# UoL-SignalProcessingGroup/SMC-NUTS

Measured on AMD Instinct MI355X. Metric: leapfrog-steps/sec, higher is better.
Workload: dtype f64

## Files before the change

### include/smcnuts_hip.h

```cpp
#ifndef SMCNUTS_HIP_H
#define SMCNUTS_HIP_H

#include <stddef.h>
#include <stdint.h>

#ifdef __cplusplus
extern "C" {
#endif

typedef struct smcn_ctx smcn_ctx;

#define SMCN_MODEL_GAUSS 0
#define SMCN_MODEL_ARMA 1
#define SMCN_MODEL_PRMWCD 2
#define SMCN_MODEL_HOST 3
#define SMCN_MODEL_GLM 4
#define SMCN_MODEL_HGLM 5
#define SMCN_MODEL_CATEGORICAL 6
#define SMCN_MODEL_ORDINAL 7
#define SMCN_MODEL_MLGLM 8
#define SMCN_MODEL_WGLM 9
#define SMCN_MODEL_OGLM 10

#define SMCN_LKERNEL_FORWARD 0
#define SMCN_LKERNEL_GAUSSIAN 1

#define SMCN_FLAG_TAPE_OVERFLOW 1

int smcn_version(void);
const char* smcn_last_error(const smcn_ctx* ctx);

int smcn_ctx_create(smcn_ctx** out, int device_id, int64_t n_particles, int64_t particle_base,
                    int model_id, const double* model_data, int64_t model_data_len);
void smcn_ctx_destroy(smcn_ctx* ctx);
int smcn_dim(const smcn_ctx* ctx);
int smcn_constrained_dim(const smcn_ctx* ctx);
int smcn_fused_transitions(const smcn_ctx* ctx);
int smcn_set_stream(smcn_ctx* ctx, void* hip_stream);
int smcn_synchronize(smcn_ctx* ctx);

int smcn_set_seed(smcn_ctx* ctx, uint64_t seed);

int smcn_set_state(smcn_ctx* ctx, const double* x, const double* logw);
int smcn_get_state(smcn_ctx* ctx, double* x, double* logw, double* wn);
int smcn_get_proposal(smcn_ctx* ctx, double* r, double* x_new, double* r_new, double* logw_new);
int smcn_set_momentum(smcn_ctx* ctx, const double* r);
int smcn_set_proposal(smcn_ctx* ctx, const double* r, const double* x_new, const double* r_new);

int smcn_target_eval(smcn_ctx* ctx, const double* x, int64_t M, double phi, double* logp,
                     double* grad, double* lpri, double* llik);
int smcn_target_constrain(smcn_ctx* ctx, const double* x, int64_t M, double* out);

int smcn_init_particles_std_normal(smcn_ctx* ctx, double phi);
int smcn_init_weights(smcn_ctx* ctx, double phi, const double* logq0);

int smcn_normalise_partials(smcn_ctx* ctx, double out[4]);
int smcn_normalise_apply(smcn_ctx* ctx, double loglik);
int smcn_normalise(smcn_ctx* ctx, double* loglik, double* ess);

int smcn_moment_sums(smcn_ctx* ctx, const double* mean_or_null, double* sums);

int smcn_resample_multinomial(smcn_ctx* ctx, const double* u, double loglik, double log_n_total,
                              int64_t iteration, int64_t* idx_out);
#define SMCN_RESAMPLE_MULTINOMIAL 0
#define SMCN_RESAMPLE_SYSTEMATIC 1
int smcn_set_resample_scheme(smcn_ctx* ctx, int scheme);
int smcn_set_wide_eval(smcn_ctx* ctx, int on);
int smcn_set_phase_paths(smcn_ctx* ctx, int on);
int smcn_set_tree_align(smcn_ctx* ctx, int n);
int smcn_get_wave_iterations(smcn_ctx* ctx, uint32_t* out, int64_t n);
int smcn_set_lane_grid(smcn_ctx* ctx, int64_t waves);
int smcn_set_lane_segments(smcn_ctx* ctx, int segments);

int smcn_set_nuts_cap(smcn_ctx* ctx, int doublings, int widen);
int smcn_nuts_parked(smcn_ctx* ctx, int64_t* parked);
int smcn_set_nuts_requeue(smcn_ctx* ctx, int doublings);

int smcn_propose_nuts(smcn_ctx* ctx, double step_size, double phi, int max_depth, double delta_max,
                      int64_t iteration, const double* tape, const int64_t* tape_off);
int smcn_get_tree_stats(smcn_ctx* ctx, int32_t* nleap, int32_t* depth, int32_t* ndraws, int32_t* flags);
int smcn_last_leapfrogs(smcn_ctx* ctx, int64_t* total);
int smcn_get_density_parts(smcn_ctx* ctx, double* lpri0, double* llik0, double* lpri1, double* llik1);

int smcn_reweight(smcn_ctx* ctx, int lkernel);
int smcn_accept_reject(smcn_ctx* ctx, double phi, const double* u, int64_t iteration);
int smcn_reweight_asymptotic(smcn_ctx* ctx, double phi_old, double phi_new);
int smcn_set_logw_density_ratio(smcn_ctx* ctx, double phi_num, double phi_den);

int smcn_set_lkernel_values(smcn_ctx* ctx, const double* L, const double* q);

int smcn_gauss_lkernel_sums(smcn_ctx* ctx, const double* shift, double* sums);
int smcn_gauss_lkernel_logpdf(smcn_ctx* ctx, const double* mu_x, const double* m0, const double* B,
                              const double* U, double c0);
int smcn_gauss_lkernel_device(smcn_ctx* ctx, double info[4]);
int smcn_gauss_lkernel_buffers(smcn_ctx* ctx, int world, void** local_dev, void** gathered_dev);
int smcn_gauss_lkernel_stage(smcn_ctx* ctx, int stage, int world, double n_total, double info[4] );

int smcn_temper_partials(smcn_ctx* ctx, double phi_old, double phi_new, double out[4]);
int smcn_temper_bisect(smcn_ctx* ctx, double phi_old, double target, double* phi, int* status);
int smcn_temper_bisect_pass(smcn_ctx* ctx, int pass, double phi_old);
int smcn_temper_bisect_buffers(smcn_ctx* ctx, int world, void** local, void** gathered);
int smcn_temper_bisect_decide(smcn_ctx* ctx, int pass, int world, double target, double phi_old);
int smcn_temper_bisect_result(smcn_ctx* ctx, double* phi, int* status);

int smcn_eval_proposed_parts(smcn_ctx* ctx, int which);

int smcn_commit(smcn_ctx* ctx, int64_t* n_moved);

int smcn_fast_begin(smcn_ctx* ctx, int64_t K, int save_history, int world);
int smcn_fast_buffers(smcn_ctx* ctx, void** local_partials, void** gathered, int* nq);
int smcn_set_resample_uniforms(smcn_ctx* ctx, const double* u);
int smcn_step_begin(smcn_ctx* ctx, int64_t k);
int smcn_step_finish(smcn_ctx* ctx, int64_t k, int world, int rank, double n_total, double step_size,
                     double phi, int max_depth, double delta_max, int lkernel, int last,
                     const double* tape, const int64_t* tape_off);
int smcn_fast_read(smcn_ctx* ctx, double* hist, double* x_saved, double* logw_saved);
int smcn_fast_read_from(smcn_ctx* ctx, double* hist, double* x_saved, double* logw_saved, int64_t k_from);
int smcn_history_download(smcn_ctx* ctx, int64_t k_from, int64_t k_to, double* x_saved, double* logw_saved);
int smcn_fuse_begin(smcn_ctx* ctx, int Bmax, int world);
int smcn_fuse_buffers(smcn_ctx* ctx, void** local_partials, void** gathered, int* nq);
int smcn_fuse_run(smcn_ctx* ctx, int64_t k0, int B, int world, int rank, double n_total, double step_size,
                  double phi, int max_depth, double delta_max, int decided);
// ... 133 lines not shown
```

### smcnuts_amd/_capi.py

```python
import ctypes as C
import os

import numpy as np

from . import build as _build

MODEL_GAUSS, MODEL_ARMA, MODEL_PRMWCD, MODEL_HOST = 0, 1, 2, 3
MODEL_GLM = 4
MODEL_HGLM = 5
MODEL_CATEGORICAL = 6
MODEL_ORDINAL = 7
MODEL_MLGLM = 8
MODEL_WGLM = 9
MODEL_OGLM = 10
HOST_TARGET_FN = C.CFUNCTYPE(C.c_int, C.c_void_p, C.c_int64, C.c_int, C.POINTER(C.c_double), C.c_int,
                             C.POINTER(C.c_double), C.POINTER(C.c_double), C.POINTER(C.c_double),
                             C.POINTER(C.c_double))
LKERNEL_FORWARD, LKERNEL_GAUSSIAN = 0, 1

_dp = C.POINTER(C.c_double)
_ip = C.POINTER(C.c_int32)
_lp = C.POINTER(C.c_int64)
_ctx = C.c_void_p

# ... 14 lines not shown
    "smcn_set_momentum": ([_ctx, _dp], C.c_int),
    "smcn_set_proposal": ([_ctx, _dp, _dp, _dp], C.c_int),
    "smcn_target_eval": ([_ctx, _dp, C.c_int64, C.c_double, _dp, _dp, _dp, _dp], C.c_int),
    "smcn_target_constrain": ([_ctx, _dp, C.c_int64, _dp], C.c_int),
    "smcn_init_particles_std_normal": ([_ctx, C.c_double], C.c_int),
    "smcn_init_weights": ([_ctx, C.c_double, _dp], C.c_int),
    "smcn_normalise_partials": ([_ctx, _dp], C.c_int),
    "smcn_normalise_apply": ([_ctx, C.c_double], C.c_int),
    "smcn_normalise": ([_ctx, _dp, _dp], C.c_int),
    "smcn_moment_sums": ([_ctx, _dp, _dp], C.c_int),
    "smcn_resample_multinomial": ([_ctx, _dp, C.c_double, C.c_double, C.c_int64, _lp], C.c_int),
    "smcn_propose_nuts": ([_ctx, C.c_double, C.c_double, C.c_int, C.c_double, C.c_int64, _dp, _lp], C.c_int),
    "smcn_get_tree_stats": ([_ctx, _ip, _ip, _ip, _ip], C.c_int),
    "smcn_last_leapfrogs": ([_ctx, _lp], C.c_int),
    "smcn_get_density_parts": ([_ctx, _dp, _dp, _dp, _dp], C.c_int),
    "smcn_set_lkernel_values": ([_ctx, _dp, _dp], C.c_int),
    "smcn_reweight": ([_ctx, C.c_int], C.c_int),
    "smcn_accept_reject": ([_ctx, C.c_double, _dp, C.c_int64], C.c_int),
    "smcn_reweight_asymptotic": ([_ctx, C.c_double, C.c_double], C.c_int),
    "smcn_set_logw_density_ratio": ([_ctx, C.c_double, C.c_double], C.c_int),
    "smcn_gauss_lkernel_sums": ([_ctx, _dp, _dp], C.c_int),
    "smcn_gauss_lkernel_logpdf": ([_ctx, _dp, _dp, _dp, _dp, C.c_double], C.c_int),
    "smcn_gauss_lkernel_device": ([_ctx, _dp], C.c_int),
    "smcn_gauss_lkernel_buffers": ([_ctx, C.c_int, C.POINTER(C.c_void_p), C.POINTER(C.c_void_p)], C.c_int),
    "smcn_gauss_lkernel_stage": ([_ctx, C.c_int, C.c_int, C.c_double, _dp], C.c_int),
    "smcn_set_nuts_cap": ([_ctx, C.c_int, C.c_int], C.c_int),
    "smcn_set_nuts_requeue": ([_ctx, C.c_int], C.c_int),
    "smcn_nuts_parked": ([_ctx, C.POINTER(C.c_int64)], C.c_int),
    "smcn_temper_partials": ([_ctx, C.c_double, C.c_double, _dp], C.c_int),
    "smcn_temper_bisect": ([_ctx, C.c_double, C.c_double, C.POINTER(C.c_double), C.POINTER(C.c_int)], C.c_int),
    "smcn_temper_bisect_pass": ([_ctx, C.c_int, C.c_double], C.c_int),
    "smcn_temper_bisect_buffers": ([_ctx, C.c_int, C.POINTER(C.c_void_p), C.POINTER(C.c_void_p)], C.c_int),
    "smcn_temper_bisect_decide": ([_ctx, C.c_int, C.c_int, C.c_double, C.c_double], C.c_int),
    "smcn_temper_bisect_result": ([_ctx, C.POINTER(C.c_double), C.POINTER(C.c_int)], C.c_int),
    "smcn_eval_proposed_parts": ([_ctx, C.c_int], C.c_int),
    "smcn_commit": ([_ctx, _lp], C.c_int),
    "smcn_fast_begin": ([_ctx, C.c_int64, C.c_int, C.c_int], C.c_int),
    "smcn_fast_buffers": ([_ctx, C.POINTER(C.c_void_p), C.POINTER(C.c_void_p), C.POINTER(C.c_int)], C.c_int),
    "smcn_set_resample_uniforms": ([_ctx, _dp], C.c_int),
    "smcn_step_begin": ([_ctx, C.c_int64], C.c_int),
    "smcn_step_finish": ([_ctx, C.c_int64, C.c_int, C.c_int, C.c_double, C.c_double, C.c_double, C.c_int,
                          C.c_double, C.c_int, C.c_int, _dp, _lp], C.c_int),
    "smcn_fast_read": ([_ctx, _dp, _dp, _dp], C.c_int),
    "smcn_fast_read_from": ([_ctx, _dp, _dp, _dp, C.c_int64], C.c_int),
    "smcn_history_download": ([_ctx, C.c_int64, C.c_int64, _dp, _dp], C.c_int),
    "smcn_fuse_begin": ([_ctx, C.c_int, C.c_int], C.c_int),
    "smcn_fuse_buffers": ([_ctx, C.POINTER(C.c_void_p), C.POINTER(C.c_void_p), C.POINTER(C.c_int)], C.c_int),
    "smcn_fuse_run": ([_ctx, C.c_int64, C.c_int, C.c_int, C.c_int, C.c_double, C.c_double, C.c_double, C.c_int,
                       C.c_double, C.c_int], C.c_int),
    "smcn_set_resample_scheme": ([_ctx, C.c_int], C.c_int),
    "smcn_set_wide_eval": ([_ctx, C.c_int], C.c_int),
    "smcn_set_phase_paths": ([_ctx, C.c_int], C.c_int),
    "smcn_set_tree_align": ([_ctx, C.c_int], C.c_int),
    "smcn_get_wave_iterations": ([_ctx, C.POINTER(C.c_uint32), C.c_int64], C.c_int),
    "smcn_set_lane_grid": ([_ctx, C.c_int64], C.c_int),
    "smcn_set_lane_segments": ([_ctx, C.c_int], C.c_int),
    "smcn_set_host_target": ([_ctx, HOST_TARGET_FN, C.c_void_p], C.c_int),
    "smcn_moment_sums_of": ([_ctx, _dp, C.c_int, _dp, _dp], C.c_int),
    "smcn_block_resample_local": ([_ctx, C.c_int64], C.c_int),
    "smcn_block_launch": ([_ctx, C.c_int64, C.c_int, C.c_double, C.c_double, C.c_int, C.c_double], C.c_int),
    "smcn_block_post": ([_ctx, C.c_int64, C.c_int, C.c_int], C.c_int),
    "smcn_block_partials_get": ([_ctx, C.c_int, _dp], C.c_int),
    "smcn_block_partials_set": ([_ctx, C.c_int, C.c_int, _dp], C.c_int),
    "smcn_block_stats": ([_ctx, C.c_int64, C.c_int, C.c_int, C.c_int, C.c_double, C.c_double, C.c_int], C.c_int),
    "smcn_block_wait": ([_ctx, C.c_int, C.POINTER(C.c_int), C.POINTER(C.c_int)], C.c_int),
    "smcn_block_commit": ([_ctx, C.c_int64, C.c_int], C.c_int),
    "smcn_set_block_post": ([_ctx, C.c_int], C.c_int),
    "smcn_block_ess": ([_ctx, C.c_int, _dp], C.c_int),
    "smcn_fuse_decide": ([_ctx, C.c_int64, C.c_int, C.c_int, C.c_double, C.c_double, C.POINTER(C.c_int)], C.c_int),
    "smcn_fuse_finish": ([_ctx, C.c_int64, C.c_int, C.c_int, C.c_int, C.c_double, C.c_double,
                          C.POINTER(C.c_int)], C.c_int),
    "smcn_partials_get": ([_ctx, _dp], C.c_int),
    "smcn_partials_set_gathered": ([_ctx, _dp, C.c_int], C.c_int),
    "smcn_timers": ([_ctx, _dp, C.c_int], C.c_int),
    "smcn_selftest_math": ([_ctx, _dp, C.c_int64, _dp], C.c_int),
    "smcn_measure_peaks": ([_ctx, _dp], C.c_int),
    "smcn_selftest_wide": ([_ctx, C.c_int, _dp, C.c_int64, _dp], C.c_int),
    "smcn_selftest_recur": ([_ctx, _dp, C.c_int64, _dp], C.c_int),
    "smcn_device_cache_trim": ([C.c_int, C.POINTER(C.c_int64), C.POINTER(C.c_int64)], C.c_int),
    "smcn_debug_profile": ([_ctx, C.POINTER(C.c_uint64), C.c_int], C.c_int),
    "smcn_bench_resample": ([_ctx, C.c_int, C.c_int64, _dp], C.c_int),
    "smcn_comm_unique_id": ([C.c_char_p], C.c_int),
    "smcn_comm_init": ([_ctx, C.c_int, C.c_int, C.c_char_p], C.c_int),
    "smcn_comm_destroy": ([_ctx], C.c_int),
    "smcn_comm_info": ([_ctx, C.POINTER(C.c_int)], C.c_int),
    "smcn_comm_allgather": ([_ctx, C.c_void_p, C.c_void_p, C.c_int64], C.c_int),
    "smcn_comm_allgather_host": ([_ctx, _dp, C.c_int64, _dp], C.c_int),
    "smcn_comm_alltoallv": ([_ctx, C.c_void_p, _lp, C.c_void_p, _lp, C.c_int], C.c_int),
    "smcn_buf_get": ([_ctx, C.c_void_p, C.c_int64, _dp], C.c_int),
    "smcn_buf_set": ([_ctx, C.c_void_p, C.c_int64, _dp], C.c_int),
    "smcn_buf_copy": ([_ctx, C.c_void_p, C.c_void_p, C.c_int64], C.c_int),
    "smcn_gres_begin": ([_ctx, C.c_int, _dp], C.c_int),
    "smcn_gres_buffers": ([_ctx] + [C.POINTER(C.c_void_p)] * 6, C.c_int),
    "smcn_gres_plan": ([_ctx, C.c_int, C.c_int, _dp, C.c_int64, _ip], C.c_int),
    "smcn_gres_set_order": ([_ctx, _ip], C.c_int),
    "smcn_gres_reserve": ([_ctx, C.c_int64], C.c_int),
    "smcn_gres_serve": ([_ctx, C.c_int, C.c_int, C.c_int64], C.c_int),
    "smcn_gres_finish": ([_ctx, C.c_int, _dp], C.c_int),
    "smcn_pointwise_dims": ([_ctx, _lp, C.POINTER(C.c_int)], C.c_int),
    "smcn_pointwise_loglik": ([_ctx, _dp, C.c_int64, _dp], C.c_int),
    "smcn_pointwise_partials": ([_ctx, _dp, _dp, C.c_int64, _dp], C.c_int),
    "smcn_pointwise_last_ms": ([_ctx, _dp], C.c_int),
    "smcn_psis_candidates": ([_ctx, _dp, _dp, C.c_int64, C.c_double, C.c_int64, _dp], C.c_int),
    "smcn_psis_body": ([_ctx, _dp, _dp, C.c_int64, C.c_double, C.c_int64, _dp, _dp], C.c_int),
    "smcn_psis_fit": ([_ctx, _dp, _dp, C.c_int64, C.c_double, C.c_int64, _dp], C.c_int),
    "smcn_psis_loo": ([_ctx, _dp, _dp, C.c_int64, _dp, _dp], C.c_int),
# ... 504 lines not shown
```

### smcnuts_amd/csrc/smcn_api.hip

```cpp
#include <hip/hip_runtime.h>

#include <dlfcn.h>

#include <cmath>
#include <cstdio>
#include <cstring>
#include <chrono>
#include <cstdlib>
#include <map>
#include <mutex>
#include <string>
#include <thread>
#include <unordered_map>
#include <vector>

#include "smcn_ctx.hpp"
#include "smcn_nuts.hpp"
#include "smcn_nuts_wave.hpp"
#include "smcn_nuts_fin.hpp"
#include "smcn_nuts2.hpp"
#include "smcn_nuts3.hpp"
#include "smcn_temper.hpp"
#include "smcn_nuts_host.hpp"
#include "smcn_weights.hpp"
// ... 441 lines not shown
    *out = c;
    return 0;
}

void smcn_ctx_destroy(smcn_ctx* c) {
    if (!c) return;
    (void)hipSetDevice(c->device);
    (void)stream_wait(c->stream);
    free_all(c);
    delete c;
}

int smcn_dim(const smcn_ctx* c) { return c ? c->D : -1; }
int smcn_constrained_dim(const smcn_ctx* c) { return c ? c->Dc : -1; }
int smcn_fused_transitions(const smcn_ctx* c) { return c ? (c->fused_ok ? 1 : 0) : -1; }

int smcn_set_stream(smcn_ctx* c, void* s) {
    CHECK_CTX(c);
    HIPC(c, stream_wait(c->stream));
    if (c->own_stream && c->stream) pool_give(c->device, c->stream);
    c->stream = (hipStream_t)s;
    c->own_stream = false;
    return 0;
}

int smcn_synchronize(smcn_ctx* c) {
    CHECK_CTX(c);
    HIPC(c, stream_wait(c->stream));
    return 0;
}

int smcn_set_resample_scheme(smcn_ctx* c, int scheme) {
    CHECK_CTX(c);
    if (scheme != 0 && scheme != 1) FAIL(c, "smcn_set_resample_scheme: 0 (multinomial) or 1 (systematic)");
    c->resample_scheme = scheme;
    return 0;
}
int smcn_set_wide_eval(smcn_ctx* c, int on) {
    CHECK_CTX(c);
    if (on != 0 && on != 1) FAIL(c, "smcn_set_wide_eval: 0 or 1");
    c->wide_eval = on;
    return 0;
}
int smcn_set_phase_paths(smcn_ctx* c, int on) {
    CHECK_CTX(c);
    if (on != 0 && on != 1) FAIL(c, "smcn_set_phase_paths: 0 or 1");
    c->phase_paths = on;
    return 0;
}
int smcn_set_tree_align(smcn_ctx* c, int n) {
    CHECK_CTX(c);
    if (n != 1 && n != 2 && n != 4 && n != 8) FAIL(c, "smcn_set_tree_align: 1, 2, 4 or 8");
    c->tree_align = n;
    return 0;
}
int smcn_get_wave_iterations(smcn_ctx* c, uint32_t* out, int64_t n) {
    CHECK_CTX(c);
    if (!out || n < 0) FAIL(c, "smcn_get_wave_iterations: bad arguments");
    if (n > c->wave_iters_n) FAIL(c, "smcn_get_wave_iterations: the last lane-kernel launch had fewer wavefronts (or there was none)");
    HIPC(c, stream_wait(c->stream));
    if (n > 0) HIPC(c, hipMemcpy(out, c->wave_iters, sizeof(uint32_t) * n, hipMemcpyDeviceToHost));
    return 0;
}
int smcn_set_block_post(smcn_ctx* c, int mode) {
    CHECK_CTX(c);
    if (mode != 0 && mode != 1) FAIL(c, "smcn_set_block_post: 0 (separate launches) or 1 (fused)");
    c->block_post_mode = mode;
    return 0;
}

int smcn_set_lane_grid(smcn_ctx* c, int64_t waves) {
    CHECK_CTX(c);
    c->lane_grid_cap = waves;
    return 0;
}

int smcn_set_lane_segments(smcn_ctx* c, int segments) {
    CHECK_CTX(c);
    if (segments < 0 || segments > 64) FAIL(c, "smcn_set_lane_segments: 0 (auto) .. 64");
    c->lane_segments = segments;
    return 0;
}

int smcn_set_host_target(smcn_ctx* c, smcn_host_target_fn fn, void* user) {
    CHECK_CTX(c);
    if (c->model != SMCN_MODEL_HOST) FAIL(c, "smcn_set_host_target: the context was not created with SMCN_MODEL_HOST");
    c->host_fn = fn;
    c->host_user = user;
    return 0;
}

int smcn_set_seed(smcn_ctx* c, uint64_t seed) {
    CHECK_CTX(c);
    c->seed = seed;
    return 0;
}

}

bool smcn_host::has_constrain_pass(const smcn_ctx* c) {
    return c->model == SMCN_MODEL_HGLM || c->model == SMCN_MODEL_ORDINAL || c->model == SMCN_MODEL_MLGLM;
}
void smcn_host::launch_constrain_pass(smcn_ctx* c, const double* x, double* out, int64_t M, int64_t Np, int64_t si,
                                      int64_t sc) {
    if (c->model == SMCN_MODEL_ORDINAL)
        ord_constrain_kernel<<<grid_for(M, 256), 256, 0, c->stream>>>(x, out, M, Np, c->D, (int)c->reg.p, si, sc);
// ... 815 lines not shown
    c->kin_valid = false;
    if (a.resume_in) {
        a.kin0 = nullptr; a.kin1 = nullptr; a.moved = nullptr;
    }
    HIPC(c, hipMemsetAsync(c->queue, 0, sizeof(unsigned int) * 16, c->stream));
    return timed_launch(c, [&] { nuts_kernel<Model, HBM, TP><<<(int)blocks, kNutsBlock, lds, c->stream>>>(a); });
}

static int reset_records(smcn_ctx* c, int64_t cap, int D) {
    c->rec_cap = 0;
    HIPC(c, stream_wait(c->stream));
    c->in_rec.release();
    c->out_rec.release();
    HIPC(c, c->in_rec.reset(c->N * cap * n2_in_doubles(D)));
    HIPC(c, c->out_rec.reset(c->N * cap * n2_out_doubles(D)));
    c->rec_cap = cap;
    return 0;
}
template <class Model, bool TAPE, int LC, int LF>
static int launch_nuts3(smcn_ctx* c, Nuts2Args a, const double* tape_d, const int64_t* tape_off_d, bool fuse_reweight,
                        int B, double* gen_x, double* gen_logw, double* cnt, int phase) {
    constexpr int D = Model::D, VP = n2_vp(D);
    const int64_t N = c->N;
    if (TAPE && B != 1) FAIL(c, "nuts3: recorded tapes replay one transition at a time");
    if (phase == 2 && B > c->rec_cap) FAIL(c, "nuts3: post without a launch");
    if (B > c->rec_cap) {
        const int cap = c->fuse_max > B ? c->fuse_max : B;
        if (int rc = reset_records(c, cap, D)) return rc;
    }
    const size_t lds = (size_t)n3_lds_bytes<Model>(LC, LF);
    int64_t blocks = (N + kN3Block - 1) / kN3Block;
    const int64_t resident = (int64_t)c->num_cu * 4;
    if (c->lane_grid_cap > 0 && blocks > c->lane_grid_cap) blocks = c->lane_grid_cap;
    else if (c->lane_grid_cap == 0 && blocks > resident) blocks = resident;
    if (((N + blocks - 1) / blocks + 63) / 64 > kN3ReadyWords) blocks = (N + kN3Block - 1) / kN3Block;
    if (int rc = grow(c, c->n2_ovf, blocks * kN3Block * 2 * (int64_t)n3_ovf_pairs(D, LC, LF))) return rc;
    a.ovf = c->n2_ovf;
    if (phase != 2) {
        if (int rc = grow(c, c->wave_iters, blocks)) return rc;
        a.wave_iters = c->wave_iters;
        a.tree_align = c->tree_align;
        c->wave_iters_n = blocks;
        if (c->momentum_set && B != 1) FAIL(c, "nuts3: caller-supplied momenta go with single transitions");
        nuts3_prep_kernel<D><<<grid_for(N * B, 256), 256, 0, c->stream>>>(c->x, c->momentum_set ? c->r : nullptr, c->r,
                                                                         c->in_rec, N, c->base, c->seed, a.iter, B, tape_d,
                                                                         tape_off_d);
        c->momentum_set = false;
        a.in = c->in_rec;
        a.out = c->out_rec;
        a.B = B;
        a.logw0 = (fuse_reweight && B > 1) ? c->logw : nullptr;
        a.wide = (c->wide_eval ? 1 : 0) | 2;
        a.phase_paths = c->phase_paths;
        const bool queued = blocks * kN3Block < N;
        a.seg_len = 0;
        a.seg_tail = 0;
        a.seg_align = 4;
        if (queued) {
            const int64_t per_wave = (N + blocks - 1) / blocks, words = (per_wave + 63) / 64;
            int nseg = c->lane_segments > 0 ? c->lane_segments : 4;
            if (nseg > B) nseg = (int)B;
            while (nseg > 1 && nseg * words > kN3ReadyWords) --nseg;
            a.seg_tail = 0;
            if (nseg > 1) a.seg_len = (int)((B + nseg - 1) / nseg);
            int64_t segs = a.seg_len > 0 ? (B + a.seg_len - 1) / a.seg_len : 1;
            const int64_t last_len = B - (segs - 1) * a.seg_len;
            if (segs > 1 && last_len >= 2 && (segs + 1) * words <= kN3ReadyWords) {
                a.seg_tail = (int)((2 * last_len + 2) / 5 > 0 ? (2 * last_len + 2) / 5 : 1);
                ++segs;
            }
            const int64_t hw = N * (segs - 1) * 2 * (n2_vp(D) / 2 + 1);
            if (int rc = grow(c, c->handover, hw)) return rc;
            a.handover = c->handover;
        }
        const void* const kfn = queued ? (const void*)nuts3_kernel<Model, TAPE, LC, LF, true, 1>
                                       : (const void*)nuts3_kernel<Model, TAPE, LC, LF, false, 1>;
        HIPC(c, hipFuncSetAttribute(kfn, hipFuncAttributeMaxDynamicSharedMemorySize, (int)lds));
        const int rc = timed_launch(c, [&] {
            if (queued) nuts3_kernel<Model, TAPE, LC, LF, true, 1><<<(int)blocks, kN3Block, lds, c->stream>>>(a);
            else nuts3_kernel<Model, TAPE, LC, LF, false, 1><<<(int)blocks, kN3Block, lds, c->stream>>>(a);
        });
        if (rc) return rc;
    }
    if (phase == 1) return 0;
    c->streamed_g = 0;
    if (const int slots = (phase == 2 && fuse_reweight && gen_x && gen_logw && cnt) ? block_stream_slots(c, B) : 0) {
        const int g = partials_grid(c, B);
        if ((int64_t)g * B * (gen_block_nq(D) + 2) > part_doubles(c->D)) FAIL(c, "nuts3: block partials do not fit");
        double* const cntpart = c->part + (int64_t)g * B * gen_block_nq(D);
        auto stream = [&](auto kr) {
            block_stream_kernel<D, decltype(kr)::value><<<dim3(g, B), kRedBlock, 0, c->stream>>>(
                c->out_rec, c->in_rec, c->x, c->logw, c->x_new, c->r_new, c->lpri0, c->llik0, c->lpri1, c->llik1,
                c->nleap, c->depth, c->ndraws, c->flags, c->logw_new, c->x_next, c->logw_next, gen_x, gen_logw, N, B,
                c->cmodel, c->part, cntpart);
        };
        if (slots == 4) stream(std::integral_constant<int, 4>{});
        else stream(std::integral_constant<int, 8>{});
        HIPC(c, hipGetLastError());
        c->streamed_g = g;
        return 0;
    }
    nuts2_post_kernel<D><<<grid_for(N, 256), 256, 0, c->stream>>>(
        c->out_rec, c->in_rec, c->x, fuse_reweight ? c->logw : nullptr, c->x_new, c->r_new, c->lpri0, c->llik0,
        c->lpri1, c->llik1, c->nleap, c->depth, c->ndraws, c->flags, fuse_reweight ? c->logw_new : nullptr, gen_x,
        gen_logw, cnt, N, c->D, VP, B, (fuse_reweight && B > 1) ? 1 : 0, 1);
    HIPC(c, hipGetLastError());
// ... 1413 lines not shown
```

### smcnuts_amd/csrc/smcn_ctx.hpp

```cpp
#pragma once
#include <hip/hip_runtime.h>

#include <chrono>
#include <cstdint>
#include <cstdlib>
#include <string>
#include <vector>

#include "../../include/smcnuts_hip.h"
#include "smcn_comm.hpp"
#include "smcn_devbuf.hpp"
#include "smcn_draw_plan.hpp"
#include "smcn_regdata.hpp"

namespace smcn { struct PwArgs; }

namespace smcn_host __attribute__((visibility("hidden"))) {
using namespace smcn;
constexpr int kTimerRing = 512;

struct CacheMem { static int alloc(void** p, size_t bytes); static void free(void* p, bool synced); };
struct PinnedMem {
    static int alloc(void** p, size_t bytes) { return (int)hipHostMalloc(p, bytes); }
    static void free(void* p, bool) { (void)hipHostFree(p); }
// ... 71 lines not shown
    bool own_stream = false;
    uint64_t seed = 0;
    std::string err;
    std::vector<double> mdata_h;
    RegLayout reg;

    Buf<double> mdata, x, x_new, x_tmp, r, r_new;
    Buf<double> logw, logw_new, wn, work;
    Buf<double> lpri0, llik0, lpri1, llik1, Lg, qv;
    Buf<double> scan_local, ttot, toff, part, scal;
    Buf<double> glk_buf;
    Buf<double> glk_xchg;
    int glk_world = 0;
    int nuts_jcap = 0, nuts_wide2 = 1;
    Buf<double> nuts_resume;
    Buf<unsigned int> nuts_pend;
    Buf<unsigned int> nuts_mq;
    Buf<double> nuts_mq_rec;
    int nuts_mq_b = 0;
    bool nuts_mq_used = false;
    bool nuts_mq_ok = false;
    int64_t nuts_parked = 0;
    Buf<double> stage;
    Buf<double> stage2;
    Buf<double> cstage;
    Buf<int32_t> nleap, depth, ndraws, flags;
    Buf<int64_t> idx;
    Buf<unsigned int> queue;
    Buf<double> kin0;
    Buf<double> kin1;
    Buf<int32_t> moved_i;
    bool kin_valid = false;
    bool r_pm = false, r_new_pm = false;
    Buf<unsigned long long> prof;
    Buf<double> tape_d;
    Buf<int64_t> tape_off_d;
    bool momentum_set = false, lg_set = false, q_set = false, u_set = false;
    Buf<double> hist, ss, lp, gath, hist_x, hist_logw;
    Buf<double> u_res;
    Buf<double> in_rec, out_rec;
    Buf<double> nuts_scratch;
    int64_t fast_K = -1;
    bool fast_hist = false;
    int fuse_max = 0;
    int64_t rec_cap = 0;
    int resample_scheme = 0;
    bool fused_ok = false;
    bool lane_kernel = false;
    int64_t arma_T = 0;
    Buf<double> tb_state, tb_part, tb_local, tb_gath;
    int tb_world = 0, tb_blocks = 0;
    int wide_eval = 1;
    int phase_paths = 1;
    int tree_align = 4;
    Buf<unsigned int> wave_iters;
    int64_t wave_iters_n = 0;
    int64_t lane_grid_cap = 0;
    int lane_segments = 0;
    Buf<unsigned long long> handover;
    bool plain_block = false;
    int block_post_mode = 1;
    bool cnt_zeroed = false;
    int streamed_g = 0;
    double block_phi = 1.0;
    struct { int64_t k0 = -1; int B = 0; double n_total = 0.0, phi = 0.0; } tail_combined;
    Buf<double> x_next, logw_next;
    uint64_t api_seq = 0;
    struct { uint64_t seq = 0; int64_t k0 = -1; int B = 0; } next;
    ncclComm_t comm = nullptr;
    int comm_rank = 0, comm_world = 1;
    Buf<double> g_ttot_all, g_toff_all, g_keys, g_keys_send, g_keys_recv, g_rows_send, g_rows_recv;
    Buf<int32_t> g_dest, g_order;
    int64_t g_serve_cap = 0;
    int g_world = 0;
    smcn_host_target_fn host_fn = nullptr;
    void* host_user = nullptr;
    Buf<double> hc_vec, hc_sc, hc_gp, hc_gl;
    Buf<int32_t> hc_st;
    std::vector<double> hx, hlp, hll, hgp, hgl;
    Buf<double> n2_ovf;
    Buf<double> ss_scratch;
    DevBuf<double, PinnedMem> rows_h;
    DevBuf<double, PinnedMem> hist_h;
    bool hist_h_valid = false;
    DevEvent<HipEv, false> ev_rows;
    hipStream_t dl_stream = nullptr;
    Buf<double> dl_stage;
    Buf<double> lpB, gathB, gen_x, gen_logw, cnt, shiftB;

    Event ev0[kTimerRing], ev1[kTimerRing];
    int ev_n = 0;
    double nuts_ms = 0.0;
    int64_t nuts_launches = 0;

    PwState pw;
    PsState ps;
    PrState pr;
    DrState dr;
    SmState sm;
    CovState cov;
    StState st;
    FcState fc;
};

#define CHECK_CTX(c)            \
    if (!(c)) return -1;         \
// ... 104 lines not shown
```

### smcnuts_amd/csrc/smcn_nuts2.hpp

```cpp
#pragma once
#include "smcn_nuts.hpp"

namespace smcn {

__host__ __device__ constexpr int n2_vp(int DL) { return (DL + 1) & ~1; }
__host__ __device__ constexpr int n2_in_doubles(int DL) { return 2 * n2_vp(DL) + 2; }
__host__ __device__ constexpr int n2_out_doubles(int DL) { return 2 * n2_vp(DL) + 6; }

struct Nuts2Args {
    int64_t N;
    int64_t particle_base;
    const double* mdata;
    const double* in;
    double* out;
    unsigned int* queue;
    double eps, phi, delta_max;
    int max_depth;
    uint64_t seed;
    uint32_t iter;
    int B;
    const double* tape;
    const int64_t* tape_off;
    unsigned long long* prof;
    double* ovf;
    const double* logw0 = nullptr;
    int seg_len = 0;
    int seg_tail = 0;
    int seg_align = 1;
    unsigned long long* handover = nullptr;
    int wide = 3;
    int phase_paths = 1;
    int tree_align = 1;
    unsigned int* wave_iters = nullptr;
};

template <int D>
__global__ void __launch_bounds__(256) nuts3_prep_kernel(const double* x, const double* r_in, double* r_out, double* in,
                                                         int64_t N, int64_t particle_base, uint64_t seed, uint32_t iter,
                                                         int B, const double* tape, const int64_t* tape_off) {
    using d2 = double __attribute__((ext_vector_type(2)));
    constexpr int VP = n2_vp(D), VH = VP / 2, IP = n2_in_doubles(D) / 2;
    const int64_t t = (int64_t)blockIdx.x * blockDim.x + threadIdx.x;
    if (t >= N * B) return;
    const int b = (int)(t / N);
    const int64_t p = t - (int64_t)b * N;
    d2* const rec = reinterpret_cast<d2*>(in) + (int64_t)b * IP * N + p;
    if (b == 0) {
#pragma unroll
        for (int k = 0; k < VH; ++k) {
            d2 v;
            v.x = x[(int64_t)(2 * k) * N + p];
            v.y = (2 * k + 1 < D) ? x[(int64_t)(2 * k + 1 < D ? 2 * k + 1 : 0) * N + p] : 0.0;
            rec[(int64_t)k * N] = v;
        }
    }
#pragma unroll
    for (int m = 0; m < VH; ++m) {
        d2 z;
        if (r_in) {
            z.x = r_in[(int64_t)(2 * m) * N + p];
            z.y = (2 * m + 1 < D) ? r_in[(int64_t)(2 * m + 1 < D ? 2 * m + 1 : 0) * N + p] : 0.0;
        } else {
            const u32x4 o = philox4x32_10({(uint32_t)m, (uint32_t)(particle_base + p), iter + (uint32_t)b, kStreamMomentum},
                                          (uint32_t)seed, (uint32_t)(seed >> 32));
            const double u1 = u53(o.a, o.b), u2 = u53(o.c, o.d);
            const double rad = sqrt(-2.0 * log1p(-u1));
            double sn, cs;
            sincospi(2.0 * u2, &sn, &cs);
            z.x = rad * cs;
            z.y = (2 * m + 1 < D) ? rad * sn : 0.0;
            if (b == B - 1) {
                r_out[(int64_t)(2 * m) * N + p] = z.x;
                if (2 * m + 1 < D) r_out[(int64_t)(2 * m + 1 < D ? 2 * m + 1 : 0) * N + p] = z.y;
            }
        }
        rec[(int64_t)(VH + m) * N] = z;
    }
    d2 e;
    if (tape) {
        const int64_t o = tape_off[p];
        e.x = (tape_off[p + 1] > o) ? tape[o] : 0.5;
    } else {
        e.x = -log1p(-philox_uniform(seed, iter + (uint32_t)b, (uint32_t)(particle_base + p), kStreamNuts, 0u));
    }
    e.y = 0.0;
// ... 105 lines not shown
```

### smcnuts_amd/csrc/smcn_nuts3.hpp

```cpp
#pragma once
#include "smcn_nuts2.hpp"
#include <type_traits>

namespace smcn {

constexpr int kN3Block = 64;
constexpr int kN3ReadyWords = 64;


__constant__ double kArmaFinishTab[24] = {
    1.4426950408889634074, 6.93147180369123816490e-01, 1.90821492927058770002e-10,
    2.08767569878680989792e-09, 2.50521083854417187751e-08, 2.75573192239858906526e-07,
    2.75573192239858906526e-06, 2.48015873015873015873e-05, 1.98412698412698412698e-04,
    1.38888888888888888889e-03, 8.33333333333333333333e-03, 4.16666666666666666667e-02,
    1.66666666666666666667e-01,
    0.70710678118654752440,
    9.52380952380952380952e-02, 1.05263157894736842105e-01, 1.17647058823529411765e-01,
    1.33333333333333333333e-01, 1.53846153846153846154e-01, 1.81818181818181818182e-01,
    2.22222222222222222222e-01, 2.85714285714285714286e-01, 4.0e-01, 6.66666666666666666667e-01};

struct ArmaLaneModel {
    static constexpr int D = 4;
    static constexpr bool HAS_WIDE = true;
    using cptr = const __attribute__((address_space(4))) double*;
// ... 657 lines not shown
            const unsigned int a0 = lo < 64u ? 64u : lo, b0 = w_count < lo + 64u ? w_count : lo + 64u;
            if (wi < w_words && b0 > a0) rm = (b0 - a0 >= 64u ? ~0ull : (1ull << (b0 - a0)) - 1ull) << (a0 - lo);
        }
        n_ready = w_count - (unsigned int)kN3Block;
    }
    PROF_DECL;
#ifdef SMCN_PROFILE
    unsigned long long iters = 0;
#endif
#ifdef SMCN_PROFILE_PHASE
    unsigned int prof_t0 = 0u;
#endif
    auto emit_record = [&](bool last, uint32_t qdone, bool ovdone, int nldone) __attribute__((always_inline)) {
        const gptr2 orec = (compact && last) ? out2 + p : out_cur;
        out_cur += out_stride;
        d2 t;
        const unsigned long long s0 = (unsigned long long)(unsigned)nldone | ((unsigned long long)(unsigned)j << 32);
#pragma unroll
        for (int k = 0; k < VH; ++k) {
            t.x = rx[2 * k];
            t.y = (2 * k + 1 < D) ? rx[2 * k + 1 < D ? 2 * k + 1 : 0] : 0.0;
            orec[k * N] = t;
        }
        PROF(12);
        if (compact && !last) {
            double k1 = 0.0;
#pragma unroll
            for (int k = 0; k < D; ++k) k1 = fma(rr[k], rr[k], k1);
            const double cst = 0.5 * D * kLog2Pi;
            const double qk = -0.5 * k0 - cst;
            const double Lk = -0.5 * k1 - cst;
            const double c1 = combine_lp(rl.x, rl.y, 1.0);
            const double c0 = combine_lp(lpri0, llik0, 1.0);
            lw = lw + c1 - c0 + Lk - qk;
            t.x = lw;
            t.y = __longlong_as_double((long long)s0);
            orec[VH * N] = t;
        } else {
#pragma unroll
            for (int k = 0; k < VH; ++k) {
                t.x = rr[2 * k];
                t.y = (2 * k + 1 < D) ? rr[2 * k + 1 < D ? 2 * k + 1 : 0] : 0.0;
                orec[(VH + k) * N] = t;
            }
            orec[2 * VH * N] = rl;
            t.x = lpri0; t.y = llik0;
            orec[(2 * VH + 1) * N] = t;
            const unsigned long long s1 = (unsigned long long)qdone | ((unsigned long long)(ovdone ? 1u : 0u) << 32);
            t.x = __longlong_as_double((long long)s0);
            t.y = __longlong_as_double((long long)s1);
            orec[(2 * VH + 2) * N] = t;
        }
    };
    unsigned int it = 0u;
    for (;; ++it) {
        PROF(7);
        if constexpr (QUEUE) {
            if (__ballot(phase != DONE || have_next || own_wait) == 0ull && n_ready == 0u) break;
        }
        const bool act = phase != DONE;
#ifdef SMCN_PROFILE_TAIL
        PROF_ON(__popcll(__ballot(act)) <= SMCN_PROFILE_TAIL);
#endif
#ifdef SMCN_PROFILE
        if (prof_on_) ++iters;
#endif
#ifdef SMCN_PROFILE_PHASE
        prof_ph_ = it & 3u;
        if (phase == INIT) prof_t0 = it;
        {
            const unsigned long long inph = __ballot(act && (prof_t0 & 3u) != 0u) == 0ull ? 1ull : 0ull;
            prof_inph_ = inph != 0ull;
            pacc_[4] += prof_ph_ == 0u ? 1ull : 0ull; pacc_[8] += prof_ph_ == 0u ? inph : 0ull;
            pacc_[5] += prof_ph_ == 1u ? 1ull : 0ull; pacc_[9] += prof_ph_ == 1u ? inph : 0ull;
            pacc_[6] += prof_ph_ == 2u ? 1ull : 0ull; pacc_[10] += prof_ph_ == 2u ? inph : 0ull;
            pacc_[7] += prof_ph_ == 3u ? 1ull : 0ull; pacc_[11] += prof_ph_ == 3u ? inph : 0ull;
        }
#endif
        if constexpr (!TAPE) {
            int need = 1;
            if (phase == LEAF) {
                const int t1 = __builtin_ctz(~(unsigned)i);
                need = (t1 >= j) ? j + 2 : t1;
            }
            need = need > 7 ? 7 : need;
            const unsigned long long am0 = __ballot(act);
            const int na0 = __popcll(am0);
            if (Model::HAS_WIDE && (a.wide & 2) != 0 && na0 <= 16) {
                const int avail = (int)(qfill - q);
                if (__ballot(act && avail < (need > 2 ? need : 2)) != 0ull) {
                    using u4 = unsigned int __attribute__((ext_vector_type(4)));
                    u4* const XU = reinterpret_cast<u4*>(XCH);
                    const int rank = (int)__builtin_amdgcn_mbcnt_hi((unsigned)(am0 >> 32), __builtin_amdgcn_mbcnt_lo((unsigned)am0, 0u));
                    if (act) {
                        u4 w;
                        w.x = qfill | ((unsigned)lane << 16); w.y = q;
                        w.z = (uint32_t)(a.particle_base + p); w.w = a.iter + (uint32_t)b;
                        XU[rank] = w;
                    }
                    wave_exchange_fence();
                    const int g4 = lane >> 2, h4 = lane & 3;
                    if (g4 < na0) {
                        const u4 w = XU[g4];
                        const uint32_t oq = w.x & 0xFFFFu, ol = w.x >> 16;
                        if ((int)(oq - w.y) + 2 * (h4 + 1) <= 8) {
                            const u32x4 o = philox4x32_10({(oq >> 1) + (uint32_t)h4, w.z, w.w, kStreamNuts}, (uint32_t)a.seed,
// ... 14 lines not shown
            if (act && (int)(qfill - q) <= 6) refill();
            for (;;) {
                const int avail = (int)(qfill - q);
                if (__ballot(act && avail < need) == 0ull) break;
                if (act && avail <= 6) refill();
            }
            }
            const uint32_t qt = q + (uint32_t)(phase == LEAF ? j : 0);
            up0 = ring_read(q); up1 = ring_read(q + 1u);
            utop = ring_read(qt); udir = ring_read(phase == LEAF ? qt + 1u : qt);
            pre_ok = (int)(qfill - qt) > 1;
        }
        PROF(0);

        const double e = dir * eps, h = dir * eps / 2;
        if (phase == LEAF) {
#pragma unroll
            for (int k = 0; k < D; ++k) r[k] = r[k] + h * g[k];
#pragma unroll
            for (int k = 0; k < D; ++k) x[k] = x[k] + e * r[k];
        }
        double lpri = 0.0, llik = 0.0, gp[D], gl[D];
#pragma unroll
        for (int k = 0; k < D; ++k) { gp[k] = 0.0; gl[k] = 0.0; }
        PROF(1);
        if constexpr (Model::HAS_WIDE) {
            const unsigned long long amask = __ballot(act);
            const int nact = __popcll(amask);
            double ss = 0.0, gm = 0.0, gb = 0.0, gt = 0.0;
            if (!wide_ok || nact > 16) {
                if (act) model.recur(x, ss, gm, gb, gt);
            } else if (nact > 8) model.template recur_wide<4>(x, act, amask, Yl, XCH, lane, ss, gm, gb, gt);
            else if (nact > 4) model.template recur_wide<8>(x, act, amask, Yl, XCH, lane, ss, gm, gb, gt);
            else if (nact > 2 || !wide_rows) model.template recur_wide<16>(x, act, amask, Yl, XCH, lane, ss, gm, gb, gt);
            else if (nact == 2) model.template recur_wide<32>(x, act, amask, Yl, XCH, lane, ss, gm, gb, gt);
            else model.template recur_wide<64>(x, act, amask, Yl, XCH, lane, ss, gm, gb, gt);
            if (act) model.finish(x, ss, gm, gb, gt, lpri, llik, gp, gl);
        } else {
            if (act) model.eval(x, lpri, llik, gp, gl);
        }
        PROF(2);
        double lp = lpri + phi * llik;
#pragma unroll
        for (int k = 0; k < D; ++k) g[k] = fma(phi, gl[k], gp[k]);
        if (!finite_d(lp)) {
            mov64(lp, -kInf);
#pragma unroll
            for (int k = 0; k < D; ++k) mov64(g[k], -kInf);
        }

        bool start_doubling = false;
        bool tree_end = false;
        const bool init = phase == INIT;
#ifdef SMCN_PROFILE_PHASE
        bool prof_park0 = false;
#endif
        if (phase == LEAF) {
            double kin = 0.0;
#pragma unroll
            for (int k = 0; k < D; ++k) r[k] = r[k] + h * g[k];
#pragma unroll
            for (int k = 0; k < D; ++k) kin = fma(r[k], r[k], kin);
            ++nleap;
            const double joint = lp - 0.5 * kin;
            int nsub = (logu < joint) ? 1 : 0;
            bool ssub = (logu - a.delta_max) >= joint;
            d2 leafl;
            leafl.x = lpri; leafl.y = llik;
            {
                const bool opens = j > 0 && (i & 1) == 0;
                const int lopen = opens ? ((i == 0) ? j : (__ffs(i) - 1)) : 0;
                if (lopen >= 1) {
                    movv(f1x, x); movv(f1r, r);
                    if (lopen >= 2) { movv(f2x, x); movv(f2r, r); }
                }
                for (int l = 3; l <= lopen; ++l)
                    with_first(l, [&](auto fp) __attribute__((always_inline)) { st_vec(fp, x); st_vec(fp + VH * 64, r); });
            }
            int csrc = -1;
            auto cand_value = [&](bool need, double (&cx)[D], double (&cr)[D], d2& cl) __attribute__((always_inline)) {
#pragma unroll
                for (int k = 0; k < D; ++k) { cx[k] = x[k]; cr[k] = r[k]; }
                cl = leafl;
                if (need && csrc >= 0) {
                    if (csrc == 0) { movv(cx, c0x); movv(cr, c0r); movd2(cl, c0l); }
                    else if (csrc == 1) { movv(cx, c1x); movv(cr, c1r); movd2(cl, c1l); }
                    else with_cand(csrc, [&](auto cp) __attribute__((always_inline)) {
                        double tx[D], tr[D];
                        ld_vec(cp, tx); ld_vec(cp + VH * 64, tr);
                        const d2 tl = cp[2 * VH * 64];
                        movv(cx, tx); movv(cr, tr); movd2(cl, tl);
                    });
                }
            };
            auto merge = [&](int m, double u, int nfirst, const double (&fx)[D], const double (&fr)[D]) __attribute__((always_inline)) {
                const int den = (nfirst + nsub) > 1 ? (nfirst + nsub) : 1;
                const bool keep = !(fma(u, (double)den, -(double)nsub) < 0.0);
                csrc = keep ? m : csrc;
                nsub += nfirst;
                double A = 0.0, B = 0.0;
#pragma unroll
                for (int k = 0; k < D; ++k) {
                    const double d = x[k] - fx[k];
                    A = fma(d, fr[k], A);
                    B = fma(d, r[k], B);
                }
                ssub = is_uturn(A, B, dir);
            };
            PROF(3);
            int m = 0, how = 0;
            auto ends = [&]() __attribute__((always_inline)) -> int {
                return ssub ? 1 : (m == j ? 2 : ((((i >> m) & 1) == 0) ? 3 : 0));
            };
            how = ends();
            const bool all_park0 = a.phase_paths != 0 && __ballot(how != 3) == 0ull;
#ifdef SMCN_PROFILE_PHASE
            prof_park0 = all_park0;
#endif
            if (all_park0) {
                movv(c0x, x); movv(c0r, r); movd2(c0l, leafl);
                n0 = nsub;
                ++i;
            } else {
                if (how == 0) {
                    double u;
                    if constexpr (TAPE) u = ring_draw(); else { u = up0; ++q; }
                    merge(0, u, n0, f1x, f1r);
                    m = 1;
                    how = ends();
                }
                if (how == 0) {
                    double u;
                    if constexpr (TAPE) u = ring_draw(); else { u = up1; ++q; }
                    merge(1, u, n1, f2x, f2r);
                    m = 2;
                    how = ends();
                }
                while (how == 0) {
                    double fx[D], fr[D];
                    const int nfirst = (int)*nst_ptr(m);
                    with_first(m + 1, [&](auto fp) __attribute__((always_inline)) { ld_vec(fp, fx); ld_vec(fp + VH * 64, fr); });
                    const double u = ring_draw();
                    merge(m, u, nfirst, fx, fr);
                    ++m;
                    how = ends();
                }
                PROF(8);
                bool done = false, stop = false, acc = false;
                if (how == 1) {
                    q += (uint32_t)__popc((unsigned)(i >> m) & ((1u << (j - m)) - 1u));
                    done = true; stop = true;
                } else if (how == 2) {
                    double u;
                    if (TAPE || !pre_ok) u = ring_draw(); else { u = utop; ++q; }
                    acc = nsub >= n || fma(u, (double)n, -(double)nsub) < 0.0;
                    double A = 0.0, B = 0.0;
#pragma unroll
                    for (int k = 0; k < D; ++k) {
                        const double d = x[k] - ex[k];
                        A = fma(d, er[k], A);
                        B = fma(d, r[k], B);
                    }
                    stop = is_uturn(A, B, dir);
                    done = true;
                }
                PROF(9);
                {
                    double cx[D], cr[D];
                    d2 cl;
                    const bool park = how == 3;
                    cand_value(park || acc, cx, cr, cl);
                    if (acc) { movv(rx, cx); movv(rr, cr); movd2(rl, cl); }
                    if (park) {
                        if (m == 0) { movv(c0x, cx); movv(c0r, cr); movd2(c0l, cl); }
                        else if (m == 1) { movv(c1x, cx); movv(c1r, cr); movd2(c1l, cl); }
                        else {
                            with_cand(m, [&](auto crec) __attribute__((always_inline)) { st_vec(crec, cx); st_vec(crec + VH * 64, cr); crec[2 * VH * 64] = cl; });
                            *nst_ptr(m) = (unsigned short)nsub;
                        }
                    }
                    n0 = (park && m == 0) ? nsub : n0;
                    n1 = (park && m == 1) ? nsub : n1;
                }
                PROF(4);
                if (!done) {
                    ++i;
                } else {
                    n += nsub;
                    ++j;
                    if (stop || j > a.max_depth) {
                        if constexpr (QUEUE) {
                            tree_end = true;
                        } else {
                            const bool more = b + 1 < a.B;
                            const int bdone = b;
                            const uint32_t qdone = q;
                            const bool ovdone = overflow;
                            const int nldone = nleap;
                            if (more) movv(x, rx);
                            phase = DONE;
                            take_record(more);
                            b = more ? bdone + 1 : b;
                            PROF(10);
                            emit_record(!more, qdone, ovdone, nldone);
                            PROF(13);
                            if (more && bdone + 2 < a.B) request();
                            if (more && ((it + 1u) & (unsigned int)(a.tree_align - 1)) != 0u) {
                                phase = DONE;
                                own_wait = true;
                            }
                        }
                    } else {
                        start_doubling = true;
                    }
                }
            }
        }
        if constexpr (QUEUE) {
            if (__ballot(tree_end || (phase == DONE && (have_next || own_wait || n_ready != 0u))) != 0ull) {
                __builtin_amdgcn_s_waitcnt(0x0F70);
                const bool idle = phase == DONE;
                const bool sd = b + 1 >= b_end;
                const bool last = tree_end && b + 1 >= a.B;
                const bool in_step = ((it + 1u) & (unsigned int)(a.seg_align - 1)) == 0u;
                const bool to_next = have_next && ((tree_end && sd) || idle);
                const bool take = to_next && in_step;
                const bool push = tree_end && have_next && sd && !last;
                const bool to_own = (tree_end && !(have_next && sd) && !last) || (idle && own_wait);
                const bool cont = to_own && in_step;
                own_wait = to_own && !in_step;
                const bool seg_done = cont && sd;
                const int bdone = b;
                const uint32_t qdone = q;
                const bool ovdone = overflow;
                const int nldone = nleap;
                if (cont) movv(x, rx);
                phase = tree_end ? (int)DONE : phase;
                take_record(cont || take);
                PROF(10);
                if (tree_end) emit_record(last, qdone, ovdone, nldone);
                const unsigned long long pm = __ballot(push);
                if (pm != 0ull) {
                    if (push) {
                        const gptr2 ho = (gptr2)a.handover + ((size_t)p * (nseg - 1) + (size_t)seg) * (VH + 1);
                        d2 t;
#pragma unroll
                        for (int k = 0; k < VH; ++k) {
                            t.x = rx[2 * k];
                            t.y = (2 * k + 1 < D) ? rx[2 * k + 1 < D ? 2 * k + 1 : 0] : 0.0;
                            ho[k] = t;
                        }
                        t.x = lw; t.y = 0.0;
                        ho[VH] = t;
                    }
                    const unsigned int ip = (unsigned int)(p - w_start);
                    const unsigned int pw = (unsigned int)(seg + 1) * w_words + (ip >> 6), pb = ip & 63u;
                    for (unsigned long long m = pm; m != 0ull; m &= m - 1ull) {
                        const int l = (int)__builtin_ctzll(m);
                        const unsigned int wu = (unsigned int)__builtin_amdgcn_readlane((int)pw, l);
                        const unsigned int bu = (unsigned int)__builtin_amdgcn_readlane((int)pb, l);
                        if ((unsigned int)lane == wu) rm |= 1ull << bu;
                    }
                    n_ready += (unsigned int)__popcll(pm);
                }
                if (take) {
#pragma unroll
                    for (int k = 0; k < D; ++k) mov64(x[k], hx_next[k]);
                    mov64(lw, lw_next);
                    if constexpr (TAPE) { toff = toff_next; tlen = tlen_next; }
// ... 116 lines not shown
```

Measured before the change: 8.527 billion.

## Add phase-dispatched fast path for second-in-four leaf merges in NUTS wave kernel

```diff
diff --git a/include/smcnuts_hip.h b/include/smcnuts_hip.h
--- a/include/smcnuts_hip.h
+++ b/include/smcnuts_hip.h
@@ -68,6 +68,7 @@
 int smcn_set_wide_eval(smcn_ctx* ctx, int on);
 int smcn_set_phase_paths(smcn_ctx* ctx, int on);
 int smcn_set_tree_align(smcn_ctx* ctx, int n);
+int smcn_set_phase_dispatch(smcn_ctx* ctx, int on);
 int smcn_get_wave_iterations(smcn_ctx* ctx, uint32_t* out, int64_t n);
 int smcn_set_lane_grid(smcn_ctx* ctx, int64_t waves);
 int smcn_set_lane_segments(smcn_ctx* ctx, int segments);
diff --git a/smcnuts_amd/_capi.py b/smcnuts_amd/_capi.py
--- a/smcnuts_amd/_capi.py
+++ b/smcnuts_amd/_capi.py
@@ -90,6 +90,7 @@
     "smcn_set_wide_eval": ([_ctx, C.c_int], C.c_int),
     "smcn_set_phase_paths": ([_ctx, C.c_int], C.c_int),
     "smcn_set_tree_align": ([_ctx, C.c_int], C.c_int),
+    "smcn_set_phase_dispatch": ([_ctx, C.c_int], C.c_int),
     "smcn_get_wave_iterations": ([_ctx, C.POINTER(C.c_uint32), C.c_int64], C.c_int),
     "smcn_set_lane_grid": ([_ctx, C.c_int64], C.c_int),
     "smcn_set_lane_segments": ([_ctx, C.c_int], C.c_int),
diff --git a/smcnuts_amd/csrc/smcn_api.hip b/smcnuts_amd/csrc/smcn_api.hip
--- a/smcnuts_amd/csrc/smcn_api.hip
+++ b/smcnuts_amd/csrc/smcn_api.hip
@@ -517,6 +517,12 @@
     CHECK_CTX(c);
     if (n != 1 && n != 2 && n != 4 && n != 8) FAIL(c, "smcn_set_tree_align: 1, 2, 4 or 8");
     c->tree_align = n;
+    return 0;
+}
+int smcn_set_phase_dispatch(smcn_ctx* c, int on) {
+    CHECK_CTX(c);
+    if (on != 0 && on != 1) FAIL(c, "smcn_set_phase_dispatch: 0 or 1");
+    c->phase_dispatch = on;
     return 0;
 }
 int smcn_get_wave_iterations(smcn_ctx* c, uint32_t* out, int64_t n) {
@@ -1438,6 +1444,7 @@
         a.logw0 = (fuse_reweight && B > 1) ? c->logw : nullptr;
         a.wide = (c->wide_eval ? 1 : 0) | 2;
         a.phase_paths = c->phase_paths;
+        a.phase_dispatch = c->phase_dispatch;
         const bool queued = blocks * kN3Block < N;
         a.seg_len = 0;
         a.seg_tail = 0;
diff --git a/smcnuts_amd/csrc/smcn_ctx.hpp b/smcnuts_amd/csrc/smcn_ctx.hpp
--- a/smcnuts_amd/csrc/smcn_ctx.hpp
+++ b/smcnuts_amd/csrc/smcn_ctx.hpp
@@ -147,6 +147,7 @@
     int tb_world = 0, tb_blocks = 0;
     int wide_eval = 1;
     int phase_paths = 1;
+    int phase_dispatch = 1;
     int tree_align = 4;
     Buf<unsigned int> wave_iters;
     int64_t wave_iters_n = 0;
diff --git a/smcnuts_amd/csrc/smcn_nuts2.hpp b/smcnuts_amd/csrc/smcn_nuts2.hpp
--- a/smcnuts_amd/csrc/smcn_nuts2.hpp
+++ b/smcnuts_amd/csrc/smcn_nuts2.hpp
@@ -31,6 +31,7 @@
     int wide = 3;
     int phase_paths = 1;
     int tree_align = 1;
+    int phase_dispatch = 1;
     unsigned int* wave_iters = nullptr;
 };
 
diff --git a/smcnuts_amd/csrc/smcn_nuts3.hpp b/smcnuts_amd/csrc/smcn_nuts3.hpp
--- a/smcnuts_amd/csrc/smcn_nuts3.hpp
+++ b/smcnuts_amd/csrc/smcn_nuts3.hpp
@@ -733,6 +733,7 @@
             orec[(2 * VH + 2) * N] = t;
         }
     };
+    const bool in_step4 = !TAPE && a.phase_dispatch != 0 && ((QUEUE ? a.seg_align : a.tree_align) & 3) == 0;
     unsigned int it = 0u;
     for (;; ++it) {
         PROF(7);
@@ -853,10 +854,15 @@
         bool start_doubling = false;
         bool tree_end = false;
         const bool init = phase == INIT;
+        const bool leaf = phase == LEAF;
 #ifdef SMCN_PROFILE_PHASE
         bool prof_park0 = false;
 #endif
-        if (phase == LEAF) {
+        int nsub = 0;
+        bool ssub = false;
+        d2 leafl;
+        leafl.x = lpri; leafl.y = llik;
+        if (leaf) {
             double kin = 0.0;
 #pragma unroll
             for (int k = 0; k < D; ++k) r[k] = r[k] + h * g[k];
@@ -864,10 +870,15 @@
             for (int k = 0; k < D; ++k) kin = fma(r[k], r[k], kin);
             ++nleap;
             const double joint = lp - 0.5 * kin;
-            int nsub = (logu < joint) ? 1 : 0;
-            bool ssub = (logu - a.delta_max) >= joint;
-            d2 leafl;
-            leafl.x = lpri; leafl.y = llik;
+            nsub = (logu < joint) ? 1 : 0;
+            ssub = (logu - a.delta_max) >= joint;
+        }
+        auto park0 = [&]() __attribute__((always_inline)) {
+            movv(c0x, x); movv(c0r, r); movd2(c0l, leafl);
+            n0 = nsub;
+            ++i;
+        };
+        auto leaf_generic = [&]() __attribute__((always_inline)) {
             {
                 const bool opens = j > 0 && (i & 1) == 0;
                 const int lopen = opens ? ((i == 0) ? j : (__ffs(i) - 1)) : 0;
@@ -919,9 +930,7 @@
             prof_park0 = all_park0;
 #endif
             if (all_park0) {
-                movv(c0x, x); movv(c0r, r); movd2(c0l, leafl);
-                n0 = nsub;
-                ++i;
+                park0();
             } else {
                 if (how == 0) {
                     double u;
@@ -1016,6 +1025,43 @@
                     }
                 }
             }
+        };
+        bool blocked = false;
+        if (in_step4 && (it & 3u) == 1u) {
+            const bool top0 = leaf && j == 0, mrg = leaf && j != 0;
+            const int den = (n0 + nsub) > 1 ? (n0 + nsub) : 1;
+            const bool keep = !(fma(up0, (double)den, -(double)nsub) < 0.0);
+            double A = 0.0, B = 0.0, At = 0.0, Bt = 0.0;
+#pragma unroll
+            for (int k = 0; k < D; ++k) {
+                const double d = x[k] - f1x[k], dt = x[k] - ex[k];
+                A = fma(d, f1r[k], A);
+                B = fma(d, r[k], B);
+                At = fma(dt, er[k], At);
+                Bt = fma(dt, r[k], Bt);
+            }
+            const bool ut0 = is_uturn(A, B, dir), end0 = is_uturn(At, Bt, dir) || j + 1 > a.max_depth || !pre_ok;
+            if (__ballot(leaf && (ssub || (mrg && ut0) || (top0 && end0))) == 0ull) {
+                blocked = true;
+                if (mrg) {
+                    ++q;
+                    n1 = nsub + n0;
+                    ++i;
+                }
+                if (mrg && keep) { movv(c1x, c0x); movv(c1r, c0r); movd2(c1l, c0l); }
+                if (mrg && !keep) { movv(c1x, x); movv(c1r, r); movd2(c1l, leafl); }
+                if (top0) {
+                    ++q;
+                    const bool acc = nsub >= n || fma(utop, (double)n, -(double)nsub) < 0.0;
+                    if (acc) { movv(rx, x); movv(rr, r); movd2(rl, leafl); }
+                    n += nsub;
+                    ++j;
+                    start_doubling = true;
+                }
+            }
+        }
+        if (!blocked) {
+            if (leaf) leaf_generic();
         }
         if constexpr (QUEUE) {
             if (__ballot(tree_end || (phase == DONE && (have_next || own_wait || n_ready != 0u))) != 0ull) {
```

Measured after the change: 8.573 billion (median of 6 runs). Within noise of the previous version (+0.5%).
